# rlglab/minizero

Hardware: AMD Instinct MI355X
Metric: self-play leaf-evals/s (9x9 Go AlphaZero n=400) (higher is better)
Workload: dtype f32; 1 GPU; BASELINE configs[1]: 9x9 Go AlphaZero, n=400, 6 blocks x 64 ch, 256 parallel games per GPU, synthetic fixed-weight net (seed 0), Dirichlet noise + random rotation + softmax-count moves (reference defaults); games_per_gpu=256, actor_num_simulation=400, pipeline_lanes=1, backend=nccl

## Files before the change

minizero_amd/csrc/pool_body.h:

```cpp
#pragma once
#include "pool.h"
#include <cfloat>
#include <climits>

#ifndef MZ_LPROF
#define MZ_LPROF(k)
#endif

namespace mz {

__device__ __forceinline__ float normalizedMean(const PoolView& v, float reward, float mean, float cnt, int player, int bsize, float lo, float hi)
{
    float value = reward + v.gamma * mean;
    if (v.value_rescale) {
        if (bsize < 2) { return 1.0f; }
        value = (value - lo) / (hi - lo);
        value = 2 * value - 1;
        value = value < -1.0f ? -1.0f : value;
        value = value > 1.0f ? 1.0f : value;
    }
    value = (player == v.flipping_player) ? -value : value;
    return (value * cnt - 0.0f) / (cnt + 0.0f);
}

// ... 49 lines not shown
                 "s_nop 1\n\t"
                 "v_max_u32_dpp %0, %0, %0 row_shr:2 row_mask:0xf bank_mask:0xf bound_ctrl:0\n\t"
                 "s_nop 1\n\t"
                 "v_max_u32_dpp %0, %0, %0 row_shr:4 row_mask:0xf bank_mask:0xf bound_ctrl:0\n\t"
                 "s_nop 1\n\t"
                 "v_max_u32_dpp %0, %0, %0 row_shr:8 row_mask:0xf bank_mask:0xf bound_ctrl:0\n\t"
                 "s_nop 1\n\t"
                 "v_max_u32_dpp %0, %0, %0 row_bcast:15 row_mask:0xa bank_mask:0xf\n\t"
                 "s_nop 1\n\t"
                 "v_max_u32_dpp %0, %0, %0 row_bcast:31 row_mask:0xc bank_mask:0xf\n\t"
                 "s_nop 1"
                 : "+v"(v));
    return static_cast<unsigned>(__builtin_amdgcn_readlane(static_cast<int>(v), 63));
}

struct LevelEval { float q, score; };
__device__ __forceinline__ LevelEval evalChild(const PoolView& v, const NodeRec& c, int cplayer, float bias, double sqrtN, double rc0, double rc1, bool* tiny)
{
    float value = c.reward + v.gamma * c.mean;
    value = (cplayer == v.flipping_player) ? -value : value;
    const float a = value * c.count - 0.0f;
    LevelEval e;
    e.q = static_cast<float>(static_cast<double>(a) * rc0);
    *tiny = (a != 0.0f) && (__builtin_fabsf(a) < 0x1p-100f);
    const float bpol = bias * c.policy;
    const double x = static_cast<double>(bpol) * sqrtN;
    const double d = static_cast<double>(1 + c.count);
    const double q0 = x * rc1;
    const double y = __builtin_fma(__builtin_fma(-d, q0, x), rc1, q0);
    e.score = static_cast<float>(y);
    return e;
}

typedef __attribute__((address_space(3))) int LdsI32;
typedef __attribute__((address_space(3))) const float LdsCFloat;
typedef __attribute__((address_space(3))) const double LdsCDbl;
constexpr int kSpecCap = 128;
constexpr int kSpecWay = 4 + 3 * kSpecCap;
constexpr int kGw = 4, kLv = 64 / kGw;
#ifndef MZ_SPEC_WAYS
#define MZ_SPEC_WAYS 16
#endif
constexpr int kSpecWays = MZ_SPEC_WAYS;
#define MZ_SPEC_WAYS_IS(n) static_assert(mz::kSpecWays == (n), "this translation unit sizes its LDS for " #n " remembered paths (pool_body.h MZ_SPEC_WAYS)")
static_assert((kSpecWays & (kSpecWays - 1)) == 0 && kSpecWays >= 2 && kSpecWays <= 64, "a power of two of at most one wave's lanes");
constexpr int kHelpSegs = 3;
constexpr int kHelpHdr = 16;
constexpr int kHelpSeg = kHelpHdr + 4 * kLv;
constexpr int kSpecHelp = kSpecWays * kSpecWay + 8;
constexpr int kSpecWords = kSpecHelp + kHelpSegs * kHelpSeg;
constexpr int kSpecNode = 4, kSpecFc = 4 + kSpecCap, kSpecNc = 4 + 2 * kSpecCap;
struct SpecMem { LdsI32* w; LdsCFloat* bias; LdsCDbl* sqrt; };

template <bool SPEC = false, class RcpPtr>
__device__ __forceinline__ void selectBody(const PoolView& v, const int* __restrict__ start, int g, int lane, RcpPtr rcp, SpecMem sm = SpecMem{nullptr, nullptr, nullptr}, int serial = 0)
{
    GNodeRec* recs = (GNodeRec*)(v.rec + size_t(g) * v.cap);
    int* path = v.path + size_t(g) * v.max_depth;
    int* pact = v.path_action + size_t(g) * v.max_depth;
    int* hact = v.host_path_action ? v.host_path_action + size_t(g) * v.max_depth : nullptr;
    MZ_GLOBAL const float* bias_tab = (MZ_GLOBAL const float*)v.bias_tab;
    MZ_GLOBAL const double* sqrt_tab = (MZ_GLOBAL const double*)v.sqrt_tab;
    LdsI32* spec = nullptr;
    auto note = [&](int d, int n, const NodeRec& r) {
        if (!SPEC || !sm.w) { return; }
        if (d == 1) {
            const int w = lane < kSpecWays ? lane : 0;
            const int lw = sm.w[w * kSpecWay], nw = sm.w[w * kSpecWay + kSpecNode + 1];
            const unsigned long long m = __ballot(lane < kSpecWays && lw > 1 && nw == n);
            int way;
            if (m != 0) {
                way = static_cast<int>(__builtin_ctzll(m));
                if (lane == 0) { sm.w[kSpecWays * kSpecWay + 3] += 1; }
            } else {
                way = __builtin_amdgcn_readfirstlane(sm.w[kSpecWays * kSpecWay]) & (kSpecWays - 1);
                if (lane == 0) { sm.w[kSpecWays * kSpecWay] = way + 1; sm.w[way * kSpecWay] = 0; }
            }
            spec = sm.w + way * kSpecWay;
            if (lane == 0) { sm.w[kSpecWays * kSpecWay + 6] = way; }
        }
        if (spec && lane == 0 && d < kSpecCap) {
            spec[kSpecNode + d] = n;
            spec[kSpecFc + d] = r.first_child;
            spec[kSpecNc + d] = r.num_children;
        }
    };
    const int bsize = v.bound_size[g];
    const float lo = v.bound_lo[g], hi = v.bound_hi[g];
    auto uniformRec = [](NodeRec r) {
        NodeRec u;
        u.count = __int_as_float(__builtin_amdgcn_readfirstlane(__float_as_int(r.count)));
        u.mean = __int_as_float(__builtin_amdgcn_readfirstlane(__float_as_int(r.mean)));
        u.policy = __int_as_float(__builtin_amdgcn_readfirstlane(__float_as_int(r.policy)));
        u.reward = __int_as_float(__builtin_amdgcn_readfirstlane(__float_as_int(r.reward)));
        u.first_child = __builtin_amdgcn_readfirstlane(r.first_child);
        u.num_children = __builtin_amdgcn_readfirstlane(r.num_children);
        u.action = __builtin_amdgcn_readfirstlane(r.action);
        u.players = __builtin_amdgcn_readfirstlane(r.players);
        return u;
    };
    NodeRec cur = uniformRec(loadRec(recs));
    int node = 0, depth = 1;
    if (lane == 0) { path[0] = 0; pact[0] = cur.action; if (hact) { hact[0] = cur.action; } }
    const int st = start ? __builtin_amdgcn_readfirstlane(start[g]) : 0;
    if (st > 0) {
        node = st;
        cur = uniformRec(loadRec(recs + st));
        if (lane == 0) { path[1] = st; pact[1] = cur.action; if (hact) { hact[1] = cur.action; } }
        note(1, st, cur);
        depth = 2;
    }
    const int max_depth = __builtin_amdgcn_readfirstlane(v.max_depth);
    for (;;) {
        cur.count = __int_as_float(__builtin_amdgcn_readfirstlane(__float_as_int(cur.count)));
        cur.first_child = __builtin_amdgcn_readfirstlane(cur.first_child);
        cur.num_children = __builtin_amdgcn_readfirstlane(cur.num_children);
        cur.players = __builtin_amdgcn_readfirstlane(cur.players);
        depth = __builtin_amdgcn_readfirstlane(depth);
        node = __builtin_amdgcn_readfirstlane(node);
        if (!(cur.num_children != 0 && depth < max_depth)) { break; }
        const int nc = cur.num_children, fc = cur.first_child, cplayer = (cur.players >> 8) & 0xFF;
        const int N = static_cast<int>(cur.count - 1);
        const float bias = bias_tab[N];
        const double sqrtN = sqrt_tab[N];
        if (nc <= 128 || (node != 0 && min(nc, static_cast<int>(static_cast<unsigned>(cur.players) >> 16) + 1) <= 128)) {
            const int ne = node == 0 ? nc : min(nc, static_cast<int>(static_cast<unsigned>(cur.players) >> 16) + 1);
            if (SPEC && spec && node != 0 && !v.atari_init_q && !v.value_rescale) {
                const int L0 = depth - 1;
                const int plen = __builtin_amdgcn_readfirstlane(spec[0]);
                if (serial > 0 && L0 > kLv && (L0 - 1) % kLv == 0 && (L0 - 1) / kLv <= kHelpSegs) {
                    LdsI32* h = sm.w + kSpecHelp + ((L0 - 1) / kLv - 1) * kHelpSeg;
                    if (__builtin_amdgcn_readfirstlane(h[0]) == serial) {
                        __builtin_amdgcn_fence(__ATOMIC_ACQUIRE, "workgroup");
                        const int hadv = __builtin_amdgcn_readfirstlane(h[3]);
                        if (__builtin_amdgcn_readfirstlane(h[2]) == node && hadv > 0 && depth + hadv <= max_depth) {
                            if (lane < hadv) {
                                const int ch = h[kHelpHdr + lane], ca = h[kHelpHdr + kLv + lane];
                                path[depth + lane] = ch;
                                pact[depth + lane] = ca;
                                if (hact) { hact[depth + lane] = ca; }
                                if (depth + lane < kSpecCap) {
                                    spec[kSpecNode + depth + lane] = ch;
                                    spec[kSpecFc + depth + lane] = h[kHelpHdr + 2 * kLv + lane];
                                    spec[kSpecNc + depth + lane] = h[kHelpHdr + 3 * kLv + lane];
                                }
                            }
                            cur.count = __int_as_float(__builtin_amdgcn_readfirstlane(h[4]));
                            cur.first_child = __builtin_amdgcn_readfirstlane(h[5]);
                            cur.num_children = __builtin_amdgcn_readfirstlane(h[6]);
                            cur.action = __builtin_amdgcn_readfirstlane(h[7]);
                            cur.players = __builtin_amdgcn_readfirstlane(h[8]);
                            node = __builtin_amdgcn_readfirstlane(h[9]);
                            depth += hadv;
                            if (lane == 0) { sm.w[kSpecWays * kSpecWay + 7] += hadv; }
                            continue;
                        }
                    }
                }
                if (L0 + 1 < plen && L0 + 1 < kSpecCap && __builtin_amdgcn_readfirstlane(spec[kSpecNode + L0]) == node) {
                    int K = plen - L0 < kSpecCap - L0 ? plen - L0 : kSpecCap - L0;
                    K = K < kLv ? K : kLv;
                    const int k = lane / kGw, j = lane % kGw, Lk = L0 + k, base8 = lane - j;
                    const bool inrange = k < K;
                    const int nk = inrange ? (k == 0 ? node : spec[kSpecNode + Lk]) : 0;
                    const int fck = inrange ? (k == 0 ? fc : spec[kSpecFc + Lk]) : 0;
                    const int nck = inrange ? (k == 0 ? nc : spec[kSpecNc + Lk]) : 0;
                    const int pfc = (inrange && k >= 1) ? (k == 1 ? fc : spec[kSpecFc + Lk - 1]) : 0;
                    const int pnc = (inrange && k >= 1) ? (k == 1 ? nc : spec[kSpecNc + Lk - 1]) : 0;
                    const int nl = nck < kGw ? nck : kGw;
                    const bool ld = inrange && j < nl;
                    const NodeRec c = loadRec(recs + (ld ? fck + j : 0));
                    const int idx = nk - pfc;
// ... 570 lines not shown
```

minizero_amd/csrc/sim.hip:

```cpp
#include "sim_az_body.h"
#include "sim_mz_body.h"

namespace mz {

MZ_SPEC_WAYS_IS(16);

template <int H, int W, int CIN0_PAD, int CDYN_PAD, int CPAD>
__global__ __launch_bounds__(512) void sim_kernel_mz(const SimArgs* __restrict__ a_, int sim0, int nsims, int host_start, int pre_epoch)
{
    CSimArgs* a = (CSimArgs*)a_;
    extern __shared__ __attribute__((aligned(16))) float tiles[];
    const int g = blockIdx.x, tid = threadIdx.x, lane = tid & 63, wave = tid >> 6;
    constexpr int CM = CIN0_PAD > CDYN_PAD ? (CIN0_PAD > CPAD ? CIN0_PAD : CPAD) : (CDYN_PAD > CPAD ? CDYN_PAD : CPAD);
    constexpr int kTileFloats = kTowerTiles * CM * planeStride(H, W);
    double* rcp_w = reinterpret_cast<double*>(tiles + kTileFloats);
    const int rcp_n = a->rcp_n;
    for (int i = tid; i < rcp_n; i += 512) { rcp_w[i] = a->pv.rcp_tab[i]; }
    LdsCDouble* rcp_lds = (LdsCDouble*)rcp_w;
    const int tab_n = rcp_n - 2;
    double* sqrt_w = rcp_w + rcp_n;
    float* bias_w = reinterpret_cast<float*>(sqrt_w + tab_n);
    int* spec_w = reinterpret_cast<int*>(bias_w + tab_n + (tab_n & 1));
    for (int i = tid; i < tab_n; i += 512) { sqrt_w[i] = a->pv.sqrt_tab[i]; bias_w[i] = a->pv.bias_tab[i]; }
    if (!a->atari) {
// ... 449 lines not shown
#ifdef MZ_SIM_TPROF
    {
        unsigned long long h[64];
        if (hipMemcpyFromSymbol(h, HIP_SYMBOL(g_tp), sizeof(h)) == hipSuccess && h[63]) {
            fprintf(stderr, "[mz sim tprof] cycles per layer (game 0, avg over %llu towers):", h[63]);
            for (int i = 0; i < 14; ++i) { fprintf(stderr, " %.0f", double(h[i]) / double(h[63])); }
            fprintf(stderr, "\n");
        }
    }
#endif
    if (sim_prof_.n == 0) { return; }
    hipLaunchKernelGGL(sim_prof_fold, dim3(1), dim3(1), 0, stream_, sim_prof_.p + sim_prof_.n - kSimProfTail);
    if (hipStreamSynchronize(stream_) != hipSuccess) { return; }
    std::vector<unsigned long long> h(sim_prof_.n);
    if (hipMemcpy(h.data(), sim_prof_.p, h.size() * sizeof(unsigned long long), hipMemcpyDeviceToHost) != hipSuccess) { return; }
    const std::vector<unsigned long long> tail(h.end() - kSimProfTail, h.end());
    h.resize(h.size() - kSimProfTail);
    double skipped = 0, skipped_max = 0, sims_all = 0;
    for (size_t g = 0; g < h.size() / 8; ++g) {
        const double sk = double(h[g * 8 + 4] >> 32);
        h[g * 8 + 4] &= 0xFFFFFFFFull;
        skipped += sk; sims_all += double(h[g * 8 + 4]);
        skipped_max = std::max(skipped_max, sk / std::max(1.0, double(h[g * 8 + 4])));
    }
    { double ps = 0, ac = 0, kk = 0; for (size_t g = 0; g < h.size() / 8; ++g) { ps += double(h[g * 8 + 7] >> 40); ac += double((h[g * 8 + 7] >> 20) & 0xFFFFF); kk += double(h[g * 8 + 7] & 0xFFFFF); } fprintf(stderr, "[mz sim prof] path speculation: %.0f passes, %.0f levels taken, %.0f walks that found a remembered path\n", ps, ac, kk); }
    const char* names[4] = {"select+leaf", "tower", "heads", "cand+expand"};
    const size_t G = h.size() / 8;
    double tot_all = 0, tot_max = 0;
    for (int k = 0; k < 4; ++k) {
        double sum = 0, mx = 0, sims = 0;
        for (size_t g = 0; g < G; ++g) { sum += double(h[g * 8 + k]); mx = std::max(mx, double(h[g * 8 + k])); sims += double(h[g * 8 + 4]); }
        fprintf(stderr, "[mz sim prof] %-12s avg %8.2f us per simulation (slowest game %8.2f us)\n", names[k], sum / std::max(1.0, sims) * 0.01,
                mx / std::max(1.0, sims / G) * 0.01);
        tot_all += sum / std::max(1.0, sims) * 0.01;
    }
    {
        double sel = 0, lev = 0, sims = 0, maxlev = 0;
        double helped = 0;
        const unsigned long long low = (1ull << 40) - 1;
        for (size_t g = 0; g < G; ++g) { sel += double(h[g * 8 + 5]); lev += double(h[g * 8 + 6] & low); helped += double(h[g * 8 + 6] >> 40); sims += double(h[g * 8 + 4]); maxlev = std::max(maxlev, double(h[g * 8 + 6] & low) / std::max(1.0, double(h[g * 8 + 4]))); }
        fprintf(stderr, "[mz sim prof] levels taken over from the helper waves: %.0f (%.1f %% of all levels)\n", helped, 100.0 * helped / std::max(1.0, lev));
        fprintf(stderr, "[mz sim prof] select alone avg %8.2f us, path length avg %.2f (deepest game avg %.2f) -> %.2f us per level\n", sel / std::max(1.0, sims) * 0.01,
                lev / std::max(1.0, sims), maxlev, sel / std::max(1.0, lev) * 0.01);
    }
    for (size_t g = 0; g < G; ++g) { tot_max = std::max(tot_max, double(h[g * 8] + h[g * 8 + 1] + h[g * 8 + 2] + h[g * 8 + 3]) / std::max(1.0, double(h[g * 8 + 4])) * 0.01); }
    fprintf(stderr, "[mz sim prof] total        avg %8.2f us per simulation (slowest game %8.2f us)\n", tot_all, tot_max);
    {
        double tw = 0, hd = 0;
        for (size_t g = 0; g < G; ++g) { tw += double(h[g * 8 + 1]); hd += double(h[g * 8 + 2]); }
        const double ran = std::max(1.0, sims_all - skipped);
        fprintf(stderr, "[mz sim prof] terminal leaves: network skipped in %.0f of %.0f simulations (%.2f %%; the game with the most: %.2f %%) -> per simulation that ran them: tower %.2f us, heads %.2f us\n",
                skipped, sims_all, 100.0 * skipped / std::max(1.0, sims_all), 100.0 * skipped_max, tw / ran * 0.01, hd / ran * 0.01);
    }
    if (tail[8] > 0) {
        const double L = double(tail[8]), first = double(tail[9]) / L * 0.01, last = double(tail[10]) / L * 0.01, mean = double(tail[11]) / L * 0.01;
        const double helping = double(tail[12]) / L * 0.01;
        fprintf(stderr, "[mz sim prof] launches: %llu, avg per launch from the first game's start: first game done %.1f us, mean %.1f us, last %.1f us -> %.1f %% of the CU time idles at the end of a launch\n",
                tail[8], first, mean, last, 100.0 * (last - mean - helping) / std::max(1e-9, last));
        if (tail[13] > 0 || tail[15] > 0) {
            double tw = 0;
            for (size_t g = 0; g < G; ++g) { tw += double(h[g * 8 + 1]); }
            const double ran = sims_all - skipped, pn = double(tail[13]), pt = double(tail[14]);
            fprintf(stderr, "[mz sim prof] tail help: %.0f of the %.0f simulations that ran the network had a pair tower (%.2f %%): tower %.2f us with a helper, %.2f us alone; %llu games helped, "
                            "a CU helps for %.1f us per launch after its own game (%.1f %% of the launch)\n",
                    pn, ran, 100.0 * pn / std::max(1.0, ran), pt / std::max(1.0, pn) * 0.01, (tw - pt) / std::max(1.0, ran - pn) * 0.01, tail[15], helping,
                    100.0 * helping / std::max(1e-9, last));
        }
    }
}

static size_t simLdsBound(size_t tile_bytes, int n, int A, size_t head_floats)
{
    const size_t rcp_n = size_t(n) + 5, max_depth = size_t(n) + 3;
    return tile_bytes + rcp_n * (2 * sizeof(double) + sizeof(float)) + kSpecWords * sizeof(int) + (size_t(5) * (A + 1) + 26 + 18 * 12 + 2 * max_depth + 2 + head_floats) * sizeof(float) +
           size_t(kGoSeenCap) * sizeof(uint64_t);
}

int Net::uploadSimArgs(const SimArgs& a)
{
    static_assert(sizeof(SimArgs) % 4 == 0, "SimArgs is copied as words");
    if (sim_args_host_.size() != sizeof(SimArgs) || memcmp(sim_args_host_.data(), &a, sizeof(SimArgs)) != 0) {
        if (!sim_args_.ensure(sizeof(SimArgs))) { setError("hipMalloc of the simulation arguments failed"); return MZ_ERR_DEVICE; }
        MZ_HIP(hipStreamSynchronize(stream_));
        MZ_HIP(hipMemcpy(sim_args_.p, &a, sizeof(SimArgs), hipMemcpyHostToDevice));
        sim_args_host_.assign(reinterpret_cast<const char*>(&a), reinterpret_cast<const char*>(&a) + sizeof(SimArgs));
    }
    return MZ_OK;
}

bool Net::hasSimKernelWide(int board_n, int env_kind, int num_simulation) const
{
    if (desc_.type != 0 || !use_fused_ || repr_.empty() || precision_ != 0) { return false; }
    HeadParams hp;
    makeHeadParams(&hp);
    GoDevView gv{};
    gv.n = board_n; gv.P = board_n * board_n; gv.W = (gv.P + 63) / 64; gv.Ppad = 64 * gv.W; gv.A = desc_.action_size;
    const int max_depth = num_simulation + 3;
    size_t scratch = std::max(std::max(goLeafSmemBytes(gv, max_depth), azCandSmemBytes(gv.A)), gumbelSmemBytes(gv.A));
    scratch = std::max(scratch, size_t(2) * (size_t(num_simulation) + 8) * sizeof(float));
    return simWidePlan(board_n, env_kind, num_simulation, hp, desc_.num_input_channels, (gv.P + 31) / 32, goLeafSmemBytes(gv, max_depth), scratch, nullptr, nullptr, nullptr);
}

bool Net::hasSimKernel(int board_n, int env_kind, int num_simulation) const
{
    if (desc_.type != 0 || !use_fused_) { return false; }
    if (hasSimKernelWide(board_n, env_kind, num_simulation)) { return true; }
// ... 372 lines not shown
```

minizero_amd/csrc/sim_az_body.h:

```cpp
#pragma once
#include "net.h"
#ifdef MZ_SIM_TPROF
__device__ unsigned long long g_tp[64];
__shared__ unsigned long long s_tp_prev;
__shared__ int s_tp_idx;
#define MZ_TPROF(slot)                                                                         \
    do {                                                                                       \
        if ((slot) == 3 && threadIdx.x == 0 && blockIdx.x == 0) {                              \
            const unsigned long long t_ = clock64();                                           \
            g_tp[s_tp_idx & 63] += t_ - s_tp_prev; s_tp_prev = t_; ++s_tp_idx;                 \
        }                                                                                      \
    } while (0)
#endif
#ifdef MZ_SIM_HPROF
#ifndef MZ_HPROF_BLOCK
#define MZ_HPROF_BLOCK 0
#endif
__device__ unsigned long long g_hp[16];
__shared__ unsigned long long s_hp_prev;
#define MZ_HPROF(k)                                                                                   \
    do {                                                                                              \
        if (threadIdx.x == 0 && blockIdx.x == MZ_HPROF_BLOCK) {                                       \
            const unsigned long long t_ = wall_clock64();                                             \
            if ((k) > 0) { g_hp[(k)] += t_ - s_hp_prev; } else { g_hp[15] += 1; }                     \
// ... 184 lines not shown
    const GoDevView gv = simLeafView(ldc(&a->gv), xchg, g);
    const PoolView pv = simPathView(ldc(&a->pv), reinterpret_cast<int*>(xchg) - 2 * a->pv.max_depth - 2, g);
    const SimXchg x{gv.A + (gv.A & 1)};
    float* sc = xchg + x.scalars();
    if (lane == 0) {
        sc[8] = gv.terminal[g] != 0 ? gv.eval[g] : sc[0];
        sc[9] = 0.0f;
    }
    waveSync();
    expandBackupBody(pv, nullptr, nullptr, nullptr, nullptr, nullptr, sc + 8 - g, sc + 9 - g, slot, a->err, g, lane, tiles, 2);
}

template <int WPE>
__device__ __forceinline__ void simCandExpandImpl(CSimArgs* __restrict__ a, int rot, int slot, int g, int lane, float* tiles, float* xchg, int part)
{
    g = __builtin_amdgcn_readfirstlane(g);
    slot = __builtin_amdgcn_readfirstlane(slot);
    rot = __builtin_amdgcn_readfirstlane(rot);
    const GoDevView gv = simLeafView(ldc(&a->gv), xchg, g);
    const PoolView pv = simPathView(ldc(&a->pv), reinterpret_cast<int*>(xchg) - 2 * a->pv.max_depth - 2, g);
    const SimXchg x{gv.A + (gv.A & 1)};
    const size_t ga = size_t(g) * gv.A;
    float* sc = xchg + x.scalars();
    int* cand_count = reinterpret_cast<int*>(sc + 1) - g;
    int* cand_player = reinterpret_cast<int*>(sc + 2) - g;
    int* cand_action = reinterpret_cast<int*>(xchg + x.caction()) - ga;
    Cand* cs = reinterpret_cast<Cand*>(tiles);
    Cand* out = cs + gv.A;
    const int k = reinterpret_cast<const int*>(sc)[1];
    if (a->cand_coop == 2) {
        if (k > 0 && k <= kCandCoopMaxW) {
            float* dense = simCandDense(tiles, gv.A);
            candScatterW(cs, out, reinterpret_cast<int*>(out + gv.A), k, 8, lane, reinterpret_cast<const int*>(dense + kCandCoopMaxW), a->err);
        }
    } else if (k > 0 && k <= kCandCoopMax && a->cand_coop) {
        float* dense = simCandDense(tiles, gv.A);
        candScatter(cs, out, reinterpret_cast<int*>(out + gv.A), k, 8, lane, reinterpret_cast<const int*>(dense + kCandCoopMax), a->err);
    }
    MZ_LPROF(8);
    azCandStore(gv, sc - g, out, k, cand_count, cand_action, xchg + x.cpolicy() - ga, xchg + x.clogit() - ga, cand_player, sc + 3 - g, sc + 4 - g, g, lane);
    waveSync();
    MZ_LPROF(9);
    expandBackupBody(pv, cand_count, cand_action, xchg + x.cpolicy() - ga, xchg + x.clogit() - ga, cand_player, sc + 3 - g, sc + 4 - g, slot, a->err, g,
                     lane, tiles, part);
    MZ_LPROF(12);
}

template <int WPE>
__device__ __noinline__ void simCandExpand(CSimArgs* __restrict__ a, int rot, int slot, int g, int lane, float* tiles, float* xchg, int part)
{
    simCandExpandImpl<WPE>(a, rot, slot, g, lane, tiles, xchg, part);
}

template <int WPE>
__device__ __noinline__ void simApplyRootNoise(CSimArgs* __restrict__ a, int g, int lane)
{
    g = __builtin_amdgcn_readfirstlane(g);
    const PoolView v = ldc(&a->pv);
    const size_t base = size_t(g) * v.cap;
    const int nc = v.rec[base].num_children;
    const size_t fc = base + v.rec[base].first_child;
    const float eps = a->noise_eps;
    for (int i = lane; i < nc; i += 64) {
        const float nz = a->root_noise[size_t(g) * v.A + i];
        if (a->noise_kind == kNoiseDirichlet) { v.rec[fc + i].policy = (1 - eps) * v.rec[fc + i].policy + eps * nz; }
        else { v.logit[fc + i] = v.logit[fc + i] + nz; }
        v.noise[fc + i] = nz;
    }
    waveSync();
}

template <int WPE>
__device__ __noinline__ void simGumbelStart(CSimArgs* __restrict__ a, int slot, bool host_start, int g, int lane, float* tiles, int* state_lds = nullptr)
{
    g = __builtin_amdgcn_readfirstlane(g);
    slot = __builtin_amdgcn_readfirstlane(slot);
    if (host_start && slot >= 1) { return; }
    int st = 0;
    if (slot >= 1 && !host_start) {
        const PoolView pv = ldc(&a->pv);
        GumbelView gum = ldc(&a->gum);
        if (state_lds) { gum.state = state_lds - size_t(g) * (3 + kGumbelMaxSample); }
        st = gumbelStepBody(pv, gum, slot, g, lane, tiles);
    }
    if (lane == 0) { a->start[g] = st; }
    waveSync();
}

template <int WPE, bool BIGA = false, bool FP = BIGA>
__device__ __forceinline__ void simHeadsImpl(CSimArgs* __restrict__ a, int g, int tid, float* tiles, const float* xtile, int xcs, int xpw, float* xchg)
{
    g = __builtin_amdgcn_readfirstlane(g);
    xcs = __builtin_amdgcn_readfirstlane(xcs);
    xpw = __builtin_amdgcn_readfirstlane(xpw);
    MZ_HPROF(0);
    const HeadParams hp = ldc(&a->hp);
    const SimXchg x{hp.A + (hp.A & 1)};
    const size_t ga = size_t(g) * hp.A;
    headsBody<BIGA, FP>(nullptr, hp, xchg + x.policy() - ga, xchg + x.logit() - ga, xchg + x.scalars() - g, nullptr, nullptr, 0, g, tid, 512, tiles, xtile, xcs, xpw);
    MZ_HPROF(1);
}
template <int WPE, bool BIGA = false, bool FP = BIGA>
__device__ __noinline__ void simHeads(CSimArgs* __restrict__ a, int g, int tid, float* tiles, const float* xtile, int xcs, int xpw, float* xchg)
{
    simHeadsImpl<WPE, BIGA, FP>(a, g, tid, tiles, xtile, xcs, xpw, xchg);
}

__device__ __forceinline__ bool simLeafTerminal(CSimArgs* __restrict__ a, const float* xchg)
{
    if (a->no_spec & 16) { return false; }
    const int A = a->gv.A;
    const SimXchg x{A + (A & 1)};
    return __builtin_amdgcn_readfirstlane(reinterpret_cast<const int*>(xchg + x.scalars())[6]) != 0;
}

constexpr int kSimProfTail = 16;
__device__ __forceinline__ void simProfEnter(unsigned long long* tail)
{
    atomicMin(tail + 0, wall_clock64() - tail[4]);
}
__device__ __forceinline__ void simProfExit(unsigned long long* tail)
{
    const unsigned long long t = wall_clock64() - tail[4];
    atomicMin(tail + 1, t);
    atomicMax(tail + 2, t);
    atomicAdd(tail + 3, t);
    atomicAdd(tail + 5, 1ull);
}

template <int H, int W, int CIN0_PAD, int CPAD, bool BF = false>
constexpr int simWavesPerEu() { return (!BF && H * W <= 64 && kTowerTiles * (CIN0_PAD > CPAD ? CIN0_PAD : CPAD) * planeStride(H, W) * 4 <= 76 * 1024) ? 4 : 2; }
template <int H, int W, int CIN0_PAD, int CPAD, bool BF>
constexpr int simTileFloats() { return BF ? towerBf16LdsBytes<H, W>(true) / 4 : kTowerTiles * (CIN0_PAD > CPAD ? CIN0_PAD : CPAD) * planeStride(H, W); }

template <int H, int W, int CIN0_PAD, int CPAD>
__device__ __noinline__ const float* simTower(CSimArgs* __restrict__ a, int g, int tid, float* tiles, float* xchg)
{
    g = __builtin_amdgcn_readfirstlane(g);
#ifdef MZ_SIM_TPROF
    if (tid == 0 && g == 0) { s_tp_prev = clock64(); s_tp_idx = 0; g_tp[63] += 1; }
#endif
    g = __builtin_amdgcn_readfirstlane(g);
    const GoDevView gv = simLeafView(ldc(&a->gv), xchg, g);
    return towerBody<H, W, CIN0_PAD, CPAD>(reinterpret_cast<const float*>(gv.feat), a->params, *(const TowerArgs*)&a->ta, nullptr, g, tid, tiles);
}

template <int H, int W>
__device__ __noinline__ const float* simTowerBf16(CSimArgs* __restrict__ a, int g, int tid, float* tiles, float* xchg)
{
    g = __builtin_amdgcn_readfirstlane(g);
    const GoDevView gv = simLeafView(ldc(&a->gv), xchg, g);
    return towerBodyBf16<H, W>(reinterpret_cast<const unsigned*>(gv.feat), a->wfrag, a->params, *(const TowerArgsBf16*)&a->tb, nullptr, g, tid,
                               reinterpret_cast<char*>(tiles));
}

template <int H, int W, int CIN0_PAD, int CPAD>
__device__ __noinline__ const float* simTowerPair(CSimArgs* __restrict__ a, int g, int tid, float* tiles, float* xchg, int seq, unsigned xseq, int* abort_lds)
{
    g = __builtin_amdgcn_readfirstlane(g);
    seq = __builtin_amdgcn_readfirstlane(seq);
    xseq = __builtin_amdgcn_readfirstlane(xseq);
    const GoDevView gv = simLeafView(ldc(&a->gv), xchg, g);
    const unsigned* bits = reinterpret_cast<const unsigned*>(gv.feat) + size_t(g) * gv.channels * gv.W32;
    unsigned* hb = a->help + size_t(g) * a->help_words;
    const int fw = gv.channels * gv.W32;
    if (tid < helpCmdUnits(fw)) {
        hpu4 u;
        u.x = bits[3 * tid];
        u.y = 3 * tid + 1 < fw ? bits[3 * tid + 1] : 0u;
// ... 83 lines not shown

template <int H, int W, int CIN0_PAD, int CPAD, int CPL, bool BF = false>
__global__ __launch_bounds__(512) __attribute__((amdgpu_waves_per_eu(simWavesPerEu<H, W, CIN0_PAD, CPAD, BF>(), 4))) void sim_kernel(const SimArgs* __restrict__ a_, const uint8_t* __restrict__ rot_tab, int sim0, int nsims, int host_start)
{
    CSimArgs* a = (CSimArgs*)a_;
    extern __shared__ __attribute__((aligned(16))) float tiles[];
    const int g = blockIdx.x, tid = threadIdx.x, lane = tid & 63, wave = tid >> 6;
    const int games = gridDim.x;
    constexpr int WPE = simWavesPerEu<H, W, CIN0_PAD, CPAD, BF>();
    constexpr int kTileFloats = simTileFloats<H, W, CIN0_PAD, CPAD, BF>();
    double* rcp_w = reinterpret_cast<double*>(tiles + kTileFloats);
    for (int i = tid; i < a->rcp_n; i += 512) { rcp_w[i] = a->pv.rcp_tab[i]; }
    __syncthreads();
    LdsCDouble* rcp_lds = (LdsCDouble*)rcp_w;
    SpecMem spec{nullptr, nullptr, nullptr};
    int* spec_w = nullptr;
    const int path_words = 2 * a->pv.max_depth + 2;
    float* xchg = reinterpret_cast<float*>(rcp_w + a->rcp_n) + path_words;
    if constexpr (WPE == 2) {
        const int tab_n = a->rcp_n - 2;
        double* sqrt_w = rcp_w + a->rcp_n;
        float* bias_w = reinterpret_cast<float*>(sqrt_w + tab_n);
        spec_w = reinterpret_cast<int*>(bias_w + tab_n + (tab_n & 1));
        for (int i = tid; i < tab_n; i += 512) { sqrt_w[i] = a->pv.sqrt_tab[i]; bias_w[i] = a->pv.bias_tab[i]; }
        if (tid < kSpecWays) { spec_w[tid * kSpecWay] = 0; }
        if (tid < 8) { spec_w[kSpecWays * kSpecWay + tid] = 0; }
        if (tid < kHelpSegs) { spec_w[kSpecHelp + tid * kHelpSeg] = 0; }
        __syncthreads();
        spec = SpecMem{(a->no_spec & 1) ? nullptr : (LdsI32*)spec_w, (LdsCFloat*)bias_w, (LdsCDbl*)sqrt_w};
        xchg = reinterpret_cast<float*>(spec_w + kSpecWords) + path_words;
    }
    const uint64_t* seen_lds = nullptr;
    if constexpr (CPL > 0 && WPE == 2) {
        uint64_t* sw = reinterpret_cast<uint64_t*>(xchg + ((simXchgWordsDev(a->gv.A, a->gv.channels, a->gv.W32) + 1) & ~1));
        for (int i = tid; i < kGoSeenCap; i += 512) { sw[i] = a->gv.snap[g].seen[i]; }
        __syncthreads();
        seen_lds = sw;
    }
    uint64_t* leaf_smem = nullptr;
    if constexpr (CPL > 0 && WPE == 2) {
        const HeadParams hp = ldc(&a->hp);
        if (hp.VH <= 256 && (hp.PC + 1) * hp.P <= 384 && hp.A <= 384 && !(a->no_spec & 8)) {
            leaf_smem = const_cast<uint64_t*>(seen_lds) + kGoSeenCap;
            uint64_t* zk = leaf_smem + goLeafKeyWord(a->gv.Ppad, a->gv.W, a->pv.max_depth);
            for (int i = tid; i < 2 * a->gv.P; i += 512) { zk[i] = a->gv.key[i]; }
            __syncthreads();
        }
    }
    unsigned long long* prof = a->prof ? a->prof + size_t(g) * 8 : nullptr;
    int* const node_count = reinterpret_cast<int*>(xchg) - 1;
    if (tid == 0) { *node_count = a->pv.num_nodes[g]; }
    if (prof && tid == 0) { simProfEnter(a->prof + size_t(games) * 8); }
    constexpr bool kHelp = !BF && WPE == 2 && CPL > 0 && pairTowerShape<H, W, CPAD>();
    __shared__ int s_help[4];
    const bool help_on = kHelp && (host_start & 2) != 0;
    unsigned* const help_blk = help_on ? a->help + size_t(g) * a->help_words : nullptr;
    unsigned help_xseq = 0;
    unsigned long long pair_n = 0, pair_t = 0;
    if (help_on && tid == 0) { s_help[0] = 0; s_help[1] = 0; hpStoreU(help_blk + kHpXcc, hpXccId()); }
    __syncthreads();
    for (int s = 0; s < nsims; ++s) {
        const int slot = sim0 + s;
        const int rot = rot_tab[size_t(s) * games + g];
        unsigned long long t0 = 0, t1 = 0, t2 = 0, t3 = 0, t4 = 0;
        if (prof) { t0 = wall_clock64(); }
        if (wave == 0) {
            if (slot == 1 && a->root_noise) { simApplyRootNoise<WPE>(a, g, lane); }
            if (a->use_gumbel) { simGumbelStart<WPE>(a, slot, s == 0 && (host_start & 1) != 0, g, lane, tiles); }
            simSelectLeaf<CPL, WPE>(a, rot, slot, g, lane, tiles, rcp_lds, spec, xchg, seen_lds, (a->no_spec & 2) ? 0 : s + 1, leaf_smem);
        } else if (WPE == 2 && wave <= kHelpSegs && spec.w && !(a->no_spec & 2)) {
            simSelectHelper(a, g, lane, wave, s + 1, rcp_lds, spec);
        } else if (kHelp && help_on && tid == 7 * 64) {
            s_help[1] = int(hpLoadU(help_blk + kHpHelper));
        }
        __syncthreads();
        const bool pair = kHelp && help_on && __builtin_amdgcn_readfirstlane(s_help[1]) != 0;
        const bool term = simLeafTerminal(a, xchg);
        if constexpr (CPL > 0) {
            if (!term) {
                simLeafPlanes<CPL>(a, rot, g, wave, lane, leaf_smem ? leaf_smem : reinterpret_cast<const uint64_t*>(tiles), xchg);
                __syncthreads();
            }
        }
        if (prof) { t1 = wall_clock64(); }
        const float* xt = nullptr;
        if (!term) {
            if constexpr (BF) { xt = simTowerBf16<H, W>(a, g, tid, tiles, xchg); }
            else if constexpr (WPE == 4) {
                const GoDevView gvt = simLeafView(ldc(&a->gv), xchg, g);
                xt = towerBody<H, W, CIN0_PAD, CPAD>(reinterpret_cast<const float*>(gvt.feat), a->params, *(const TowerArgs*)&a->ta, nullptr, g, tid, tiles);
            }
            else if constexpr (kHelp) {
                if (pair) {
                    xt = simTowerPair<H, W, CIN0_PAD, CPAD>(a, g, tid, tiles, xchg, s + 1, help_xseq, s_help);
                    if (!xt) { return; }
                    help_xseq += unsigned(a->ta.nlayers);
                }
                else { xt = simTower<H, W, CIN0_PAD, CPAD>(a, g, tid, tiles, xchg); }
            }
            else { xt = simTower<H, W, CIN0_PAD, CPAD>(a, g, tid, tiles, xchg); }
        }
        __syncthreads();
        if (prof) { t2 = wall_clock64(); }
        if constexpr (WPE == 4) { if (!term) { simHeadsImpl<WPE>(a, g, tid, tiles, xt, planeStride(H, W), W + 2, xchg); } }
        else if (leaf_smem && wave >= 6) { simLeafRest<CPL>(a, rot, slot, g, lane, xchg, seen_lds, leaf_smem, 7 - wave); }
        else if (!term) { simHeads<WPE, false, (MZ_HEADS_FP != 0)>(a, g, tid, tiles, xt, planeStride(H, W), W + 2, xchg); }
        else if (leaf_smem) { __syncthreads(); __syncthreads(); }
        __syncthreads();
        if (prof) { t3 = wall_clock64(); }
        if (wave == 0) { simCandGather<WPE>(a, rot, g, lane, tiles, xchg); }
        __syncthreads();
        {
            const int A = a->gv.A;
            const SimXchg x{A + (A & 1)};
            if (a->cand_coop) { simCandRank(A, reinterpret_cast<const int*>(xchg + x.scalars())[1], wave, lane, tiles); }
        }
        __syncthreads();
        {
            const bool split = !a->pv.value_rescale;
            if (wave == 0) { simCandExpand<WPE>(a, rot, slot, g, lane, tiles, xchg, split ? 1 : 0); }
            else if (wave == 1 && split) { simBackupOnly<WPE>(a, slot, g, lane, tiles, xchg); }
        }
        __syncthreads();
        if (prof && tid == 0) {
            t4 = wall_clock64();
            prof[0] += t1 - t0 + (term ? t3 - t1 : 0); prof[1] += term ? 0 : t2 - t1; prof[2] += term ? 0 : t3 - t2; prof[3] += t4 - t3;
            prof[4] += 1 + (static_cast<unsigned long long>(term) << 32);
            if (pair && !term) { pair_n += 1; pair_t += t2 - t1; }
        }
        if (kHelp && help_on && tid == 0) { hpStoreU(help_blk + kHpProgress, unsigned(s) + 1u); }
    }
    if (tid == 0) { a->pv.num_nodes[g] = *node_count; }
    if (prof && tid == 0) {
        simProfExit(a->prof + size_t(games) * 8);
        if (pair_n) { atomicAdd(a->prof + size_t(games) * 8 + 13, pair_n); atomicAdd(a->prof + size_t(games) * 8 + 14, pair_t); }
    }
    if (prof && tid == 0 && spec_w) {
        prof[7] += (static_cast<unsigned long long>(spec_w[kSpecWays * kSpecWay + 1]) << 40) | (static_cast<unsigned long long>(spec_w[kSpecWays * kSpecWay + 5]) << 20) | spec_w[kSpecWays * kSpecWay + 3];
        prof[6] += static_cast<unsigned long long>(spec_w[kSpecWays * kSpecWay + 7]) << 40;
    }
    if constexpr (kHelp) {
        if (help_on) {
            const int A = a->gv.A;
            const SimXchg x{A + (A & 1)};
            __syncthreads();
            simHelpTail<H, W, CIN0_PAD, CPAD>(a, g, tid, tiles, reinterpret_cast<unsigned*>(xchg + x.feat()), nsims, s_help);
        }
    }
}


}
```

Before: 1.616 million leaf-evals/s.

## Overlap next simulation's tree walk with candidate expansion via value-first backup

Reorders each simulation so wave 0 backs up the value first and then starts the next selection walk immediately. Waves 4-7 gather, rank, and expand the candidates of the previous leaf in parallel, and LDS flag words with polling waits replace several block-wide barriers. The walk joins (waits) only if it reaches the previous leaf before its expansion is published. This hides the expansion latency behind selection, at the cost of spin-waiting, extra synchronisation complexity, and possible stale child counts during the walk.

```diff
diff --git a/minizero_amd/csrc/pool_body.h b/minizero_amd/csrc/pool_body.h
--- a/minizero_amd/csrc/pool_body.h
+++ b/minizero_amd/csrc/pool_body.h
@@ -125,8 +125,16 @@
 constexpr int kSpecNode = 4, kSpecFc = 4 + kSpecCap, kSpecNc = 4 + 2 * kSpecCap;
 struct SpecMem { LdsI32* w; LdsCFloat* bias; LdsCDbl* sqrt; };
 
-template <bool SPEC = false, class RcpPtr>
-__device__ __forceinline__ void selectBody(const PoolView& v, const int* __restrict__ start, int g, int lane, RcpPtr rcp, SpecMem sm = SpecMem{nullptr, nullptr, nullptr}, int serial = 0)
+struct SelectJoin {
+    LdsI32* word;
+    LdsI32* stats;
+    int want, leaf, poll_limit, code;
+    int* err;
+};
+
+template <bool SPEC = false, bool JOIN = false, class RcpPtr>
+__device__ __forceinline__ void selectBody(const PoolView& v, const int* __restrict__ start, int g, int lane, RcpPtr rcp, SpecMem sm = SpecMem{nullptr, nullptr, nullptr}, int serial = 0,
+                                           SelectJoin join = SelectJoin{nullptr, nullptr, 0, -1, 0, 0, nullptr})
 {
     GNodeRec* recs = (GNodeRec*)(v.rec + size_t(g) * v.cap);
     int* path = v.path + size_t(g) * v.max_depth;
@@ -191,6 +199,31 @@
         cur.players = __builtin_amdgcn_readfirstlane(cur.players);
         depth = __builtin_amdgcn_readfirstlane(depth);
         node = __builtin_amdgcn_readfirstlane(node);
+        if constexpr (JOIN) {
+            if (node == join.leaf) {
+                join.leaf = -1;
+                int seen = __builtin_amdgcn_readfirstlane(__hip_atomic_load(join.word, __ATOMIC_RELAXED, __HIP_MEMORY_SCOPE_WORKGROUP));
+                if (seen < join.want) {
+                    const unsigned long long tw = wall_clock64();
+                    for (int i = 0; i < join.poll_limit && seen < join.want; ++i) {
+                        __builtin_amdgcn_s_sleep(1);
+                        seen = __builtin_amdgcn_readfirstlane(__hip_atomic_load(join.word, __ATOMIC_RELAXED, __HIP_MEMORY_SCOPE_WORKGROUP));
+                    }
+                    if (lane == 0) {
+                        if (seen < join.want) { atomicExch(join.err, join.code); }
+                        join.stats[1] += 1;
+                        join.stats[2] += static_cast<int>(wall_clock64() - tw);
+                    }
+                }
+                __builtin_amdgcn_fence(__ATOMIC_ACQUIRE, "workgroup");
+                if (lane == 0) { join.stats[0] += 1; }
+                cur = uniformRec(loadRec(recs + node));
+                if (SPEC && spec && lane == 0 && depth - 1 < kSpecCap) {
+                    spec[kSpecFc + depth - 1] = cur.first_child;
+                    spec[kSpecNc + depth - 1] = cur.num_children;
+                }
+            }
+        }
         if (!(cur.num_children != 0 && depth < max_depth)) { break; }
         const int nc = cur.num_children, fc = cur.first_child, cplayer = (cur.players >> 8) & 0xFF;
         const int N = static_cast<int>(cur.count - 1);
diff --git a/minizero_amd/csrc/sim.hip b/minizero_amd/csrc/sim.hip
--- a/minizero_amd/csrc/sim.hip
+++ b/minizero_amd/csrc/sim.hip
@@ -525,6 +525,9 @@
         fprintf(stderr, "[mz sim prof] terminal leaves: network skipped in %.0f of %.0f simulations (%.2f %%; the game with the most: %.2f %%) -> per simulation that ran them: tower %.2f us, heads %.2f us\n",
                 skipped, sims_all, 100.0 * skipped / std::max(1.0, sims_all), 100.0 * skipped_max, tw / ran * 0.01, hd / ran * 0.01);
     }
+    fprintf(stderr, "[mz sim prof] value first: %llu of %.0f simulations in the new order; %llu walks arrived at the previous simulation's leaf, %llu waited there (avg %.2f us); "
+                    "%llu waits at the join in front of the leaf\n",
+            tail[16], sims_all, tail[17], tail[18], double(tail[19]) / std::max(1.0, double(tail[18])) * 0.01, tail[20]);
     if (tail[8] > 0) {
         const double L = double(tail[8]), first = double(tail[9]) / L * 0.01, last = double(tail[10]) / L * 0.01, mean = double(tail[11]) / L * 0.01;
         const double helping = double(tail[12]) / L * 0.01;
diff --git a/minizero_amd/csrc/sim_az_body.h b/minizero_amd/csrc/sim_az_body.h
--- a/minizero_amd/csrc/sim_az_body.h
+++ b/minizero_amd/csrc/sim_az_body.h
@@ -260,6 +260,118 @@
     simCandExpandImpl<WPE>(a, rot, slot, g, lane, tiles, xchg, part);
 }
 
+constexpr int kVfBackup = 4;
+constexpr int kVfLeaf = 5;
+constexpr int kVfGather = 7;
+constexpr int kVfRank = 8;
+constexpr int kVfExpand = 9;
+constexpr int kVfStats = 10;
+constexpr int kVfWords = 16;
+constexpr int kVfErr = 97;
+
+__device__ __forceinline__ bool vfWait(LdsI32* w, int want, int* err, int lane)
+{
+    int seen = __builtin_amdgcn_readfirstlane(__hip_atomic_load(w, __ATOMIC_RELAXED, __HIP_MEMORY_SCOPE_WORKGROUP));
+    const bool waited = seen < want;
+    for (int i = 0; i < kHpPollLimit && seen < want; ++i) {
+        __builtin_amdgcn_s_sleep(1);
+        seen = __builtin_amdgcn_readfirstlane(__hip_atomic_load(w, __ATOMIC_RELAXED, __HIP_MEMORY_SCOPE_WORKGROUP));
+    }
+    if (seen < want && lane == 0) { atomicExch(err, kVfErr); }
+    __builtin_amdgcn_fence(__ATOMIC_ACQUIRE, "workgroup");
+    return waited;
+}
+__device__ __forceinline__ void vfPublish(LdsI32* w, int serial, int lane)
+{
+    __builtin_amdgcn_fence(__ATOMIC_RELEASE, "workgroup");
+    __builtin_amdgcn_wave_barrier();
+    if (lane == 0) { __hip_atomic_store(w, serial, __ATOMIC_RELAXED, __HIP_MEMORY_SCOPE_WORKGROUP); }
+}
+
+template <class RcpPtr>
+__device__ __noinline__ void simWalkVf(CSimArgs* __restrict__ a, int g, int lane, RcpPtr rcp, SpecMem spec, float* xchg, int serial, int join_leaf, int join_want, int* vf_)
+{
+    serial = __builtin_amdgcn_readfirstlane(serial);
+    g = __builtin_amdgcn_readfirstlane(g);
+    join_leaf = __builtin_amdgcn_readfirstlane(join_leaf);
+    join_want = __builtin_amdgcn_readfirstlane(join_want);
+    LdsI32* vf = (LdsI32*)vf_;
+    unsigned long long t0 = 0;
+    if (a->prof) { t0 = wall_clock64(); }
+    const PoolView pv = simPathView(ldc(&a->pv), reinterpret_cast<int*>(xchg) - 2 * a->pv.max_depth - 2, g);
+    selectBody<true, true>(pv, nullptr, g, lane, rcp, spec, serial, SelectJoin{vf + kVfExpand, vf + kVfStats, join_want, join_leaf, kHpPollLimit, kVfErr, a->err});
+    waveSync();
+    if (a->prof && lane == 0) {
+        a->prof[size_t(g) * 8 + 5] += wall_clock64() - t0;
+        a->prof[size_t(g) * 8 + 6] += pv.path_len[g];
+    }
+}
+
+template <int CPL>
+__device__ __noinline__ void simLeafVf(CSimArgs* __restrict__ a, int rot, int slot, int g, int lane, float* xchg, const uint64_t* seen_lds, uint64_t* leaf_smem, int* vf)
+{
+    g = __builtin_amdgcn_readfirstlane(g);
+    slot = __builtin_amdgcn_readfirstlane(slot);
+    rot = __builtin_amdgcn_readfirstlane(rot);
+    if constexpr (CPL > 0) {
+        const PoolView pv = simPathView(ldc(&a->pv), reinterpret_cast<int*>(xchg) - 2 * a->pv.max_depth - 2, g);
+        const GoDevView gv = simLeafView(ldc(&a->gv), xchg, g);
+        if (lane == 0) {
+            const int len = pv.path_len[g];
+            vf[kVfLeaf] = len > 0 ? (pv.path + size_t(g) * pv.max_depth)[len - 1] : 0;
+            vf[kVfLeaf + 1] = len > 0 ? 1 : 0;
+        }
+        leafBody<CPL, true, 1>(gv, pv, rot, slot, g, lane, leaf_smem, seen_lds);
+    }
+}
+
+template <int WPE>
+__device__ __noinline__ void simCandPipeVf(CSimArgs* __restrict__ a, int rot, int slot, int g, int lane, int w, int serial, float* tiles, float* xchg, int* vf_)
+{
+    g = __builtin_amdgcn_readfirstlane(g);
+    w = __builtin_amdgcn_readfirstlane(w);
+    serial = __builtin_amdgcn_readfirstlane(serial);
+    LdsI32* vf = (LdsI32*)vf_;
+    const int A = a->gv.A;
+    const SimXchg x{A + (A & 1)};
+    if (w == 0) {
+        simCandGatherImpl<WPE>(a, rot, g, lane, tiles, xchg);
+        vfPublish(vf + kVfGather, serial, lane);
+    } else {
+        vfWait(vf + kVfGather, serial, a->err, lane);
+    }
+    const int k = __builtin_amdgcn_readfirstlane(reinterpret_cast<const int*>(xchg + x.scalars())[1]);
+    float* dense = simCandDense(tiles, A);
+    if (k > 0 && k <= kCandCoopMax && a->cand_coop) {
+        candRankPart(dense, k, w, 8, lane, reinterpret_cast<int*>(dense + kCandCoopMax));
+        candRankPart(dense, k, w + 4, 8, lane, reinterpret_cast<int*>(dense + kCandCoopMax));
+    }
+    if (w != 0) {
+        __builtin_amdgcn_fence(__ATOMIC_RELEASE, "workgroup");
+        __builtin_amdgcn_wave_barrier();
+        if (lane == 0) { __hip_atomic_fetch_add(vf + kVfRank, 1, __ATOMIC_RELAXED, __HIP_MEMORY_SCOPE_WORKGROUP); }
+        return;
+    }
+    vfWait(vf + kVfRank, 3 * serial, a->err, lane);
+    slot = __builtin_amdgcn_readfirstlane(slot);
+    const GoDevView gv = simLeafView(ldc(&a->gv), xchg, g);
+    PoolView pv = simPathView(ldc(&a->pv), reinterpret_cast<int*>(xchg) - 2 * a->pv.max_depth - 2, g);
+    pv.path = vf_ + kVfLeaf - size_t(g) * pv.max_depth;
+    pv.path_len = vf_ + kVfLeaf + 1 - g;
+    const size_t ga = size_t(g) * gv.A;
+    float* sc = xchg + x.scalars();
+    int* cand_count = reinterpret_cast<int*>(sc + 1) - g;
+    int* cand_player = reinterpret_cast<int*>(sc + 2) - g;
+    int* cand_action = reinterpret_cast<int*>(xchg + x.caction()) - ga;
+    Cand* cs = reinterpret_cast<Cand*>(tiles);
+    Cand* out = cs + gv.A;
+    if (k > 0 && k <= kCandCoopMax && a->cand_coop) { candScatter(cs, out, reinterpret_cast<int*>(out + gv.A), k, 8, lane, reinterpret_cast<const int*>(dense + kCandCoopMax), a->err); }
+    azCandStore(gv, sc - g, out, k, cand_count, cand_action, xchg + x.cpolicy() - ga, xchg + x.clogit() - ga, cand_player, sc + 3 - g, sc + 4 - g, g, lane);
+    waveSync();
+    expandBackupBody(pv, cand_count, cand_action, xchg + x.cpolicy() - ga, xchg + x.clogit() - ga, cand_player, sc + 3 - g, sc + 4 - g, slot, a->err, g, lane, tiles, 1);
+    vfPublish(vf + kVfExpand, serial, lane);
+}
+
 template <int WPE>
 __device__ __noinline__ void simApplyRootNoise(CSimArgs* __restrict__ a, int g, int lane)
 {
@@ -322,7 +434,7 @@
     return __builtin_amdgcn_readfirstlane(reinterpret_cast<const int*>(xchg + x.scalars())[6]) != 0;
 }
 
-constexpr int kSimProfTail = 16;
+constexpr int kSimProfTail = 24;
 __device__ __forceinline__ void simProfEnter(unsigned long long* tail)
 {
     atomicMin(tail + 0, wall_clock64() - tail[4]);
@@ -512,19 +624,43 @@
     if (tid == 0) { *node_count = a->pv.num_nodes[g]; }
     if (prof && tid == 0) { simProfEnter(a->prof + size_t(games) * 8); }
     constexpr bool kHelp = !BF && WPE == 2 && CPL > 0 && pairTowerShape<H, W, CPAD>();
-    __shared__ int s_help[4];
+    __shared__ int s_help[kHelp ? kVfWords : 4];
     const bool help_on = kHelp && (host_start & 2) != 0;
     unsigned* const help_blk = help_on ? a->help + size_t(g) * a->help_words : nullptr;
     unsigned help_xseq = 0;
     unsigned long long pair_n = 0, pair_t = 0;
     if (help_on && tid == 0) { s_help[0] = 0; s_help[1] = 0; hpStoreU(help_blk + kHpXcc, hpXccId()); }
+    bool vf = false;
+    if constexpr (kHelp) {
+        vf = leaf_smem != nullptr && !a->use_gumbel && !a->pv.value_rescale && a->cand_coop != 2 && !(a->no_spec & 64);
+        if (tid >= kVfBackup && tid < kVfWords) { s_help[tid] = 0; }
+    }
+    unsigned long long vf_t0 = 0, vf_n = 0;
     __syncthreads();
     for (int s = 0; s < nsims; ++s) {
         const int slot = sim0 + s;
         const int rot = rot_tab[size_t(s) * games + g];
         unsigned long long t0 = 0, t1 = 0, t2 = 0, t3 = 0, t4 = 0;
-        if (prof) { t0 = wall_clock64(); }
-        if (wave == 0) {
+        if (prof) { t0 = (vf && s > 0) ? vf_t0 : wall_clock64(); }
+        if (kHelp && vf) {
+            if constexpr (kHelp) {
+                if (wave == 0) {
+                    if (s == 0) {
+                        if (slot == 1 && a->root_noise) { simApplyRootNoise<WPE>(a, g, lane); }
+                        simWalkVf(a, g, lane, rcp_lds, spec, xchg, (a->no_spec & 2) ? 0 : 1, -1, 0, s_help);
+                    } else {
+                        const bool waited = vfWait((LdsI32*)s_help + kVfExpand, s, a->err, lane);
+                        if (prof && waited && lane == 0) { s_help[kVfStats + 3] += 1; }
+                        if (help_on && lane == 0) { hpStoreU(help_blk + kHpProgress, unsigned(s)); }
+                    }
+                    simLeafVf<CPL>(a, rot, slot, g, lane, xchg, seen_lds, leaf_smem, s_help);
+                } else if (s == 0 && wave <= kHelpSegs && spec.w && !(a->no_spec & 2)) {
+                    simSelectHelper(a, g, lane, wave, 1, rcp_lds, spec);
+                } else if (help_on && tid == 7 * 64) {
+                    s_help[1] = int(hpLoadU(help_blk + kHpHelper));
+                }
+            }
+        } else if (wave == 0) {
             if (slot == 1 && a->root_noise) { simApplyRootNoise<WPE>(a, g, lane); }
             if (a->use_gumbel) { simGumbelStart<WPE>(a, slot, s == 0 && (host_start & 1) != 0, g, lane, tiles); }
             simSelectLeaf<CPL, WPE>(a, rot, slot, g, lane, tiles, rcp_lds, spec, xchg, seen_lds, (a->no_spec & 2) ? 0 : s + 1, leaf_smem);
@@ -568,6 +704,38 @@
         else if (leaf_smem) { __syncthreads(); __syncthreads(); }
         __syncthreads();
         if (prof) { t3 = wall_clock64(); }
+        if (kHelp && vf) {
+            if constexpr (kHelp) {
+                const bool more = s + 1 < nsims;
+                if (wave == 0) {
+                    simBackupOnly<WPE>(a, slot, g, lane, tiles, xchg);
+                    vfPublish((LdsI32*)s_help + kVfBackup, s + 1, lane);
+                    if (prof && tid == 0) {
+                        t4 = wall_clock64();
+                        prof[0] += t1 - t0 + (term ? t3 - t1 : 0); prof[1] += term ? 0 : t2 - t1; prof[2] += term ? 0 : t3 - t2; prof[3] += t4 - t3;
+                        prof[4] += 1 + (static_cast<unsigned long long>(term) << 32);
+                        if (pair && !term) { pair_n += 1; pair_t += t2 - t1; }
+                        vf_n += 1;
+                    }
+                    vf_t0 = t4;
+                    if (more) {
+                        if (slot + 1 == 1 && a->root_noise) {
+                            vfWait((LdsI32*)s_help + kVfExpand, s + 1, a->err, lane);
+                            simApplyRootNoise<WPE>(a, g, lane);
+                        }
+                        simWalkVf(a, g, lane, rcp_lds, spec, xchg, (a->no_spec & 2) ? 0 : s + 2, __builtin_amdgcn_readfirstlane(s_help[kVfLeaf]), s + 1, s_help);
+                    }
+                } else if (wave <= kHelpSegs) {
+                    if (more && spec.w && !(a->no_spec & 2)) {
+                        vfWait((LdsI32*)s_help + kVfBackup, s + 1, a->err, lane);
+                        simSelectHelper(a, g, lane, wave, s + 2, rcp_lds, spec);
+                    }
+                } else {
+                    simCandPipeVf<WPE>(a, rot, slot, g, lane, wave - 4, s + 1, tiles, xchg, s_help);
+                }
+            }
+            continue;
+        }
         if (wave == 0) { simCandGather<WPE>(a, rot, g, lane, tiles, xchg); }
         __syncthreads();
         {
@@ -589,6 +757,17 @@
             if (pair && !term) { pair_n += 1; pair_t += t2 - t1; }
         }
         if (kHelp && help_on && tid == 0) { hpStoreU(help_blk + kHpProgress, unsigned(s) + 1u); }
+    }
+    if constexpr (kHelp) {
+        if (vf) {
+            __syncthreads();
+            if (help_on && tid == 0) { hpStoreU(help_blk + kHpProgress, unsigned(nsims)); }
+            if (prof && tid == 0) {
+                unsigned long long* ptail = a->prof + size_t(games) * 8;
+                atomicAdd(ptail + 16, vf_n);
+                for (int i = 0; i < 4; ++i) { atomicAdd(ptail + 17 + i, static_cast<unsigned long long>(s_help[kVfStats + i])); }
+            }
+        }
     }
     if (tid == 0) { a->pv.num_nodes[g] = *node_count; }
     if (prof && tid == 0) {
```

New measurement: 1.644 million leaf-evals/s (median of 6 runs). 1.02x the previous value.
